# sangminwoo/SVOL

Hardware: AMD Instinct MI355X
Metric: frames/sec (fwd+matcher+bwd), T=32·P=196·d=256 (higher is better)
Workload: dtype bf16

## Files before the change

### svol_amd/csrc/gemm_ws_bf16.hip

```cpp
#include "gemm_call.h"

namespace {

struct WsArgs {
    const h16_t* A; const h16_t* W; void* C;
    const float* bias; const float* colscale; h16_t* pre; const void* res; const h16_t* aux; float* colsum;
    int64_t lda, ldw, ldc, ldp, ldr, ldaux;
    int M, N, act, tiles_per_wg, nchunk;
};

typedef __attribute__((address_space(3))) void* lds_void_ptr;

constexpr int WS_K = 256;
constexpr int TR = 16;
constexpr int A_PLANE = TR * WS_K * 2;

typedef unsigned u32x4_t __attribute__((ext_vector_type(4)));

template <int N> __device__ __forceinline__ void ws_wait_vm() { asm volatile("s_waitcnt vmcnt(%0)" ::"n"(N) : "memory"); }
__device__ __forceinline__ void ws_wait_vm_dyn(int n) {
    switch (n) {
#define C_(x) case x: ws_wait_vm<x>(); break;
        C_(0) C_(1) C_(2) C_(3) C_(4) C_(5) C_(6) C_(7) C_(8) C_(9) C_(10) C_(11) C_(12) C_(13) C_(14) C_(15) C_(16)
        C_(17) C_(18) C_(19) C_(20) C_(21) C_(22) C_(23) C_(24) C_(25) C_(26) C_(27) C_(28) C_(29) C_(30) C_(31) C_(32)
#undef C_
        default: ws_wait_vm<32>(); break;
    }
}

__device__ __forceinline__ int ws_col(int t, int i) { return (t >> 1) * 32 + (i >> 2) * 8 + (t & 1) * 4 + (i & 3); }

template <int MODE> struct WsCfg;
template <> struct WsCfg<0> { static constexpr int SLOT = A_PLANE, STG = 4, ND = 2; };
template <> struct WsCfg<1> { static constexpr int SLOT = A_PLANE + TR * 256 * 4, STG = 3, ND = 6; };
template <> struct WsCfg<2> { static constexpr int SLOT = 2 * A_PLANE, STG = 4, ND = 4; };

template <int MODE>
__device__ __forceinline__ void gemm_ws_body(const WsArgs& p) {
    constexpr int SLOT = WsCfg<MODE>::SLOT, STG = WsCfg<MODE>::STG, ND = WsCfg<MODE>::ND;
    __shared__ __attribute__((aligned(1024))) char smem[STG * SLOT];
    const int tid = threadIdx.x, lane = tid & 63;
    const int wave = __builtin_amdgcn_readfirstlane(tid >> 6);
    const int fr = lane & 15, fq = lane >> 4;
    const int chunk_id = blockIdx.x % p.nchunk, cg = blockIdx.x / p.nchunk;
    const int cg0 = cg * 256;
    const int c0 = cg0 + wave * 64;
    const bool active = c0 < p.N;
    const int tile0 = chunk_id * p.tiles_per_wg;
    const int row_base = tile0 * TR;
    const int rows_here = min(p.tiles_per_wg * TR, p.M - row_base);
    const int ntile = (rows_here + TR - 1) / TR;
    const int ns = !active ? 0 : (MODE == 0 ? (p.pre ? 4 : 2) : (MODE == 1 ? 4 : 2));

    const __amdgpu_buffer_rsrc_t rA = __builtin_amdgcn_make_buffer_rsrc(
        (void*)(p.A + (int64_t)row_base * p.lda), 0, (int)((((int64_t)rows_here - 1) * p.lda + WS_K) * 2), 0x00020000);
    int voffA[2];
#pragma unroll
    for (int j = 0; j < 2; ++j) {
        const int row = (wave * 2 + j) * 2 + (lane >> 5), s = lane & 31;
        voffA[j] = (int)(((int64_t)row * p.lda + ((s ^ row) & 31) * 8) * 2);
    }
    __amdgpu_buffer_rsrc_t rX = rA;
    int voffX[4] = {0, 0, 0, 0};
    if constexpr (MODE == 1) {
        const float* R = reinterpret_cast<const float*>(p.res) + (int64_t)row_base * p.ldr + cg0;
        const int cols = min(256, p.N - cg0);
        rX = __builtin_amdgcn_make_buffer_rsrc((void*)R, 0, (int)((((int64_t)rows_here - 1) * p.ldr + cols) * 4), 0x00020000);
#pragma unroll
        for (int j = 0; j < 4; ++j) {
            const int row = wave * 4 + j, s = lane;
            voffX[j] = (int)(((int64_t)row * p.ldr + (((s & 48) | ((s ^ row) & 15))) * 4) * 4);
        }
    } else if constexpr (MODE == 2) {
        const h16_t* X = p.aux + (int64_t)row_base * p.ldaux + cg0;
        const int cols = min(256, p.N - cg0);
        rX = __builtin_amdgcn_make_buffer_rsrc((void*)X, 0, (int)((((int64_t)rows_here - 1) * p.ldaux + cols) * 2), 0x00020000);
#pragma unroll
        for (int j = 0; j < 2; ++j) {
            const int row = (wave * 2 + j) * 2 + (lane >> 5), s = lane & 31;
            voffX[j] = (int)(((int64_t)row * p.ldaux + ((s ^ row) & 31) * 8) * 2);
        }
    }
    auto issue = [&](int slot, int tile) {
        char* sl = smem + slot * SLOT;
        const int soA = (int)((int64_t)tile * TR * p.lda * 2);
#pragma unroll
        for (int j = 0; j < 2; ++j)
            __builtin_amdgcn_raw_ptr_buffer_load_lds(rA, (lds_void_ptr)(sl + (wave * 2 + j) * 1024), 16, voffA[j], soA, 0, 0);
        if constexpr (MODE == 1) {
            const int so = (int)((int64_t)tile * TR * p.ldr * 4);
#pragma unroll
            for (int j = 0; j < 4; ++j)
                __builtin_amdgcn_raw_ptr_buffer_load_lds(rX, (lds_void_ptr)(sl + A_PLANE + (wave * 4 + j) * 1024), 16, voffX[j], so, 0, 0);
        } else if constexpr (MODE == 2) {
            const int so = (int)((int64_t)tile * TR * p.ldaux * 2);
#pragma unroll
            for (int j = 0; j < 2; ++j)
                __builtin_amdgcn_raw_ptr_buffer_load_lds(rX, (lds_void_ptr)(sl + A_PLANE + (wave * 2 + j) * 1024), 16, voffX[j], so, 0, 0);
        }
    };

    uint4 wf[4][8];
#pragma unroll
    for (int t = 0; t < 4; ++t) {
        const h16_t* wrow = p.W + (int64_t)(c0 + ws_col(t, fr)) * p.ldw + fq * 8;
#pragma unroll
        for (int ks = 0; ks < 8; ++ks) wf[t][ks] = active ? *reinterpret_cast<const uint4*>(wrow + ks * 32) : make_uint4(0, 0, 0, 0);
    }
    float bias8[2][8], scale8[2][8];
#pragma unroll
    for (int hf = 0; hf < 2; ++hf)
#pragma unroll
        for (int e = 0; e < 8; ++e) {
            const int n = c0 + hf * 32 + fq * 8 + e;
            bias8[hf][e] = (active && p.bias) ? p.bias[n] : 0.f;
            scale8[hf][e] = (MODE == 0 && active && p.colscale) ? p.colscale[n] : 1.f;
        }
    float csum[2][8];
#pragma unroll
    for (int hf = 0; hf < 2; ++hf)
#pragma unroll
        for (int e = 0; e < 8; ++e) csum[hf][e] = 0.f;

    const unsigned lds0 = (unsigned)(size_t)(lds_void_ptr)smem;
    const unsigned aoff = (unsigned)(fr * 512 + ((fq ^ fr) & 3) * 16);

#pragma unroll
    for (int s = 0; s < STG - 1; ++s)
        if (s < ntile) issue(s, s);

    for (int j = 0; j < ntile; ++j) {
        ws_wait_vm_dyn(ND * min(STG - 2, ntile - 1 - j) + ns * min(j, STG - 1));
        __builtin_amdgcn_s_barrier();
        if (j + STG - 1 < ntile) issue((j + STG - 1) % STG, j + STG - 1);
        const unsigned sl = lds0 + (unsigned)((j % STG) * SLOT);
        uint4 af[8];
        {
            const unsigned b = sl + aoff;
            const unsigned x = (unsigned)((fr & 12) * 16);
            asm volatile(
                "ds_read_b128 %0, %8\n\t"
                "ds_read_b128 %1, %9\n\t"
                "ds_read_b128 %2, %10\n\t"
                "ds_read_b128 %3, %11\n\t"
                "ds_read_b128 %4, %8 offset:256\n\t"
                "ds_read_b128 %5, %9 offset:256\n\t"
                "ds_read_b128 %6, %10 offset:256\n\t"
                "ds_read_b128 %7, %11 offset:256\n\t"
                "s_waitcnt lgkmcnt(0)"
                : "=&v"(af[0]), "=&v"(af[1]), "=&v"(af[2]), "=&v"(af[3]), "=&v"(af[4]), "=&v"(af[5]), "=&v"(af[6]), "=&v"(af[7])
                : "v"(b + ((0u * 64) ^ x)), "v"(b + ((1u * 64) ^ x)), "v"(b + ((2u * 64) ^ x)), "v"(b + ((3u * 64) ^ x))
                : "memory");
        }
        f32x4 acc[4];
#pragma unroll
        for (int t = 0; t < 4; ++t) acc[t] = f32x4{0.f, 0.f, 0.f, 0.f};
#pragma unroll
        for (int ks = 0; ks < 8; ++ks)
#pragma unroll
            for (int t = 0; t < 4; ++t)
                acc[t] = SVOL_MFMA_16x16x32_H16(__builtin_bit_cast(h16x8, wf[t][ks]),
                                                                 __builtin_bit_cast(h16x8, af[ks]), acc[t], 0, 0, 0);
        const int m = row_base + j * TR + fr;
        float v[2][8];
#pragma unroll
        for (int hf = 0; hf < 2; ++hf)
#pragma unroll
            for (int e = 0; e < 8; ++e) v[hf][e] = acc[2 * hf + (e >> 2)][e & 3];
        if constexpr (MODE == 0) {
#pragma unroll
            for (int hf = 0; hf < 2; ++hf)
#pragma unroll
                for (int e = 0; e < 8; ++e) v[hf][e] = (v[hf][e] + bias8[hf][e]) * scale8[hf][e];
            if (active && m < p.M) {
                if (p.pre) {
#pragma unroll
                    for (int hf = 0; hf < 2; ++hf) {
                        h16x8 o;
#pragma unroll
                        for (int e = 0; e < 8; ++e) o[e] = (h16_t)pre_save_fast(v[hf][e], p.act);
                        *reinterpret_cast<h16x8*>(p.pre + (int64_t)m * p.ldp + c0 + hf * 32 + fq * 8) = o;
// ... 106 lines not shown
template <int MODE, int ACT, bool PRE, bool SCALE, int VPM>
__device__ __forceinline__ void gemm_wsp_body(const WsArgs& p) {
    static_assert(MODE == 0 || MODE == 2, "bf16 outputs only");
    constexpr int SLOT = WsCfg<MODE>::SLOT, STG = 4, ND = WsCfg<MODE>::ND;
    constexpr int NS = MODE == 0 ? (PRE ? 4 : 2) : 2;
    __shared__ __attribute__((aligned(1024))) char smem[STG * SLOT];
    const int tid = threadIdx.x, lane = tid & 63;
    const int wave = __builtin_amdgcn_readfirstlane(tid >> 6);
    const int fr = lane & 15, fq = lane >> 4;
    const int chunk_id = blockIdx.x % p.nchunk, cg = blockIdx.x / p.nchunk;
    const int cg0 = cg * 256;
    const int c0 = cg0 + wave * 64;
    const bool active = c0 < p.N;
    const int tile0 = chunk_id * p.tiles_per_wg;
    const int row_base = tile0 * TR;
    const int rows_here = min(p.tiles_per_wg * TR, p.M - row_base);
    const int ntile = (rows_here + TR - 1) / TR;

    const __amdgpu_buffer_rsrc_t rA = __builtin_amdgcn_make_buffer_rsrc(
        (void*)(p.A + (int64_t)row_base * p.lda), 0, (int)((((int64_t)rows_here - 1) * p.lda + WS_K) * 2), 0x00020000);
    int voffA[2];
#pragma unroll
    for (int j = 0; j < 2; ++j) {
        const int row = (wave * 2 + j) * 2 + (lane >> 5), s = lane & 31;
        voffA[j] = (int)(((int64_t)row * p.lda + ((s ^ row) & 31) * 8) * 2);
    }
    __amdgpu_buffer_rsrc_t rX = rA;
    int voffX[2] = {0, 0};
    if constexpr (MODE == 2) {
        const h16_t* X = p.aux + (int64_t)row_base * p.ldaux + cg0;
        const int cols = min(256, p.N - cg0);
        rX = __builtin_amdgcn_make_buffer_rsrc((void*)X, 0, (int)((((int64_t)rows_here - 1) * p.ldaux + cols) * 2), 0x00020000);
#pragma unroll
        for (int j = 0; j < 2; ++j) {
            const int row = (wave * 2 + j) * 2 + (lane >> 5), s = lane & 31;
            voffX[j] = (int)(((int64_t)row * p.ldaux + ((s ^ row) & 31) * 8) * 2);
        }
    }
    auto issue = [&](int slot, int tile) {
        char* sl = smem + slot * SLOT;
        const int soA = (int)((int64_t)tile * TR * p.lda * 2);
#pragma unroll
        for (int j = 0; j < 2; ++j)
            __builtin_amdgcn_raw_ptr_buffer_load_lds(rA, (lds_void_ptr)(sl + (wave * 2 + j) * 1024), 16, voffA[j], soA, 0, 0);
        if constexpr (MODE == 2) {
            const int so = (int)((int64_t)tile * TR * p.ldaux * 2);
#pragma unroll
            for (int j = 0; j < 2; ++j)
                __builtin_amdgcn_raw_ptr_buffer_load_lds(rX, (lds_void_ptr)(sl + A_PLANE + (wave * 2 + j) * 1024), 16, voffX[j], so, 0, 0);
        }
    };

    uint4 wf[4][8];
#pragma unroll
    for (int t = 0; t < 4; ++t) {
        const h16_t* wrow = p.W + (int64_t)(c0 + ws_col(t, fr)) * p.ldw + fq * 8;
#pragma unroll
        for (int ks = 0; ks < 8; ++ks) wf[t][ks] = active ? *reinterpret_cast<const uint4*>(wrow + ks * 32) : make_uint4(0, 0, 0, 0);
    }
    float bias8[2][8], scale8[2][8];
#pragma unroll
    for (int hf = 0; hf < 2; ++hf)
#pragma unroll
        for (int e = 0; e < 8; ++e) {
            const int n = c0 + hf * 32 + fq * 8 + e;
            bias8[hf][e] = (MODE == 0 && active && p.bias) ? p.bias[n] : 0.f;
            scale8[hf][e] = (MODE == 0 && SCALE && active && p.colscale) ? p.colscale[n] : 1.f;
        }
    float csum[2][8];
#pragma unroll
    for (int hf = 0; hf < 2; ++hf)
#pragma unroll
        for (int e = 0; e < 8; ++e) csum[hf][e] = 0.f;

    const unsigned lds0 = (unsigned)(size_t)(lds_void_ptr)smem;
    const unsigned aoff = (unsigned)(fr * 512 + ((fq ^ fr) & 3) * 16);
    const unsigned ax_x = (unsigned)((fr & 12) * 16);
    const unsigned xq0 = (unsigned)(A_PLANE + fr * 512 + (((wave * 8 + fq) ^ fr) & 31) * 16);
    const unsigned xq1 = (unsigned)(A_PLANE + fr * 512 + (((wave * 8 + 4 + fq) ^ fr) & 31) * 16);
    const __amdgpu_buffer_rsrc_t rC = __builtin_amdgcn_make_buffer_rsrc(
        (void*)(reinterpret_cast<h16_t*>(p.C) + (int64_t)row_base * p.ldc), 0,
        active ? (int)((((int64_t)rows_here - 1) * p.ldc + p.N) * 2) : 0, 0x00020000);
    const __amdgpu_buffer_rsrc_t rP = __builtin_amdgcn_make_buffer_rsrc(
        (void*)(PRE ? p.pre + (int64_t)row_base * p.ldp : nullptr), 0,
        (PRE && active) ? (int)((((int64_t)rows_here - 1) * p.ldp + p.N) * 2) : 0, 0x00020000);
    const int voffC = (int)(((int64_t)fr * p.ldc + c0 + fq * 8) * 2), voffP = (int)(((int64_t)fr * p.ldp + c0 + fq * 8) * 2);
    const int cstep = (int)(TR * p.ldc * 2), pstep = (int)(TR * p.ldp * 2);

    u32x4_t af[8], ax[2] = {u32x4_t{0, 0, 0, 0}, u32x4_t{0, 0, 0, 0}};
    auto read_frags = [&](int slot) {
        const unsigned sl = lds0 + (unsigned)(slot * SLOT);
        const unsigned b = sl + aoff;
        asm volatile(
            "ds_read_b128 %0, %8\n\t"
            "ds_read_b128 %1, %9\n\t"
            "ds_read_b128 %2, %10\n\t"
            "ds_read_b128 %3, %11\n\t"
            "ds_read_b128 %4, %8 offset:256\n\t"
            "ds_read_b128 %5, %9 offset:256\n\t"
            "ds_read_b128 %6, %10 offset:256\n\t"
            "ds_read_b128 %7, %11 offset:256"
            : "=&v"(af[0]), "=&v"(af[1]), "=&v"(af[2]), "=&v"(af[3]), "=&v"(af[4]), "=&v"(af[5]), "=&v"(af[6]), "=&v"(af[7])
            : "v"(b + ((0u * 64) ^ ax_x)), "v"(b + ((1u * 64) ^ ax_x)), "v"(b + ((2u * 64) ^ ax_x)), "v"(b + ((3u * 64) ^ ax_x))
            : "memory");
        if constexpr (MODE == 2) {
            asm volatile(
                "ds_read_b128 %0, %2\n\t"
                "ds_read_b128 %1, %3"
                : "=&v"(ax[0]), "=&v"(ax[1])
                : "v"(sl + xq0), "v"(sl + xq1)
                : "memory");
        }
// ... 15 lines not shown
    };
    auto epilogue = [&](int j, const f32x4 (&acc)[4], const u32x4_t (&axj)[2]) {
        float v[2][8];
#pragma unroll
        for (int hf = 0; hf < 2; ++hf)
#pragma unroll
            for (int e = 0; e < 8; ++e) v[hf][e] = acc[2 * hf + (e >> 2)][e & 3];
        if constexpr (MODE == 0) {
#pragma unroll
            for (int hf = 0; hf < 2; ++hf)
#pragma unroll
                for (int e = 0; e < 8; ++e) {
                    v[hf][e] += bias8[hf][e];
                    if constexpr (SCALE) v[hf][e] *= scale8[hf][e];
                }
            if constexpr (PRE) {
                h16x8 o[2];
#pragma unroll
                for (int hf = 0; hf < 2; ++hf)
#pragma unroll
                    for (int e = 0; e < 8; ++e) o[hf][e] = (h16_t)pre_save_fast(v[hf][e], ACT);
                store_b128_guarded(__builtin_bit_cast(u32x4_t, o[0]), rP, voffP, j * pstep);
                store_b128_guarded(__builtin_bit_cast(u32x4_t, o[1]), rP, voffP + 64, j * pstep);
            }
            h16x8 o[2];
#pragma unroll
            for (int hf = 0; hf < 2; ++hf)
#pragma unroll
                for (int e = 0; e < 8; ++e) {
                    float y = v[hf][e];
                    if constexpr (ACT == SVOL_ACT_GELU || ACT == SVOL_ACT_GELU_D) y = gelu_fast(y);
                    if constexpr (ACT == SVOL_ACT_RELU) y = fmaxf(y, 0.f);
                    o[hf][e] = (h16_t)y;
                }
            store_b128_guarded(__builtin_bit_cast(u32x4_t, o[0]), rC, voffC, j * cstep);
            store_b128_guarded(__builtin_bit_cast(u32x4_t, o[1]), rC, voffC + 64, j * cstep);
        } else {
            h16x8 o[2];
#pragma unroll
            for (int hf = 0; hf < 2; ++hf) {
                const h16x8 a8 = __builtin_bit_cast(h16x8, axj[hf]);
#pragma unroll
                for (int e = 0; e < 8; ++e) {
                    const float d = v[hf][e] * dact_fast((float)a8[e], ACT);
                    csum[hf][e] += d;
                    o[hf][e] = (h16_t)d;
                }
            }
            store_b128_guarded(__builtin_bit_cast(u32x4_t, o[0]), rC, voffC, j * cstep);
            store_b128_guarded(__builtin_bit_cast(u32x4_t, o[1]), rC, voffC + 64, j * cstep);
        }
    };

#pragma unroll
    for (int s = 0; s < STG; ++s)
        if (s < ntile) issue(s, s);
    ws_wait_vm_dyn(ND * min(STG - 1, ntile - 1));
    __builtin_amdgcn_s_barrier();
    read_frags(0);
    wait_frags();
    f32x4 acc[4];
    mfma_slab(acc);
    for (int j = 0; j + 1 < ntile; ++j) {
        const int nd = min(STG - 2, ntile - 2 - j), nst = min(j, STG - 1);
        if (nd == STG - 2 && nst == STG - 1) ws_wait_vm<ND * (STG - 2) + NS * (STG - 1)>();
        else ws_wait_vm_dyn(ND * nd + NS * nst);
        __builtin_amdgcn_s_barrier();
        if (j + STG < ntile) issue(j % STG, j + STG);
        f32x4 accp[4];
        u32x4_t axp[2];
#pragma unroll
        for (int t = 0; t < 4; ++t) accp[t] = acc[t];
        axp[0] = ax[0];
        axp[1] = ax[1];
        read_frags((j + 1) % STG);
        wait_frags();
        mfma_slab(acc);
        epilogue(j, accp, axp);
#pragma unroll
        for (int i = 0; i < 32; ++i) {
            __builtin_amdgcn_sched_group_barrier(0x008, 1, 0);
            __builtin_amdgcn_sched_group_barrier(0x002, VPM, 0);
        }
    }
    {
        u32x4_t axp[2] = {ax[0], ax[1]};
        epilogue(ntile - 1, acc, axp);
    }
    if constexpr (MODE == 2) {
        if (p.colsum) {
#pragma unroll
            for (int hf = 0; hf < 2; ++hf)
#pragma unroll
                for (int e = 0; e < 8; ++e) {
                    float s = csum[hf][e];
                    s += __shfl_xor(s, 1, 64);
                    s += __shfl_xor(s, 2, 64);
                    s += __shfl_xor(s, 4, 64);
                    s += __shfl_xor(s, 8, 64);
                    if (fr == 0 && active) atomicAdd(p.colsum + c0 + hf * 32 + fq * 8 + e, s);
                }
        }
    }
}

#define WSP_KERNEL(name, MODE, ACT, PRE, SCALE, VPM) \
    __global__ __launch_bounds__(256, 2) void name(WsArgs p) { gemm_wsp_body<MODE, ACT, PRE, SCALE, VPM>(p); }
WSP_KERNEL(gemm_wsp_bf16_none, 0, SVOL_ACT_NONE, false, false, 2)
WSP_KERNEL(gemm_wsp_bf16_none_scale, 0, SVOL_ACT_NONE, false, true, 2)
WSP_KERNEL(gemm_wsp_bf16_gelu, 0, SVOL_ACT_GELU, false, false, 7)
WSP_KERNEL(gemm_wsp_bf16_gelu_pre, 0, SVOL_ACT_GELU, true, false, 8)
WSP_KERNEL(gemm_wsp_bf16_gelu_dpre, 0, SVOL_ACT_GELU_D, true, false, 9)
WSP_KERNEL(gemm_wsp_bf16_relu, 0, SVOL_ACT_RELU, false, false, 2)
WSP_KERNEL(gemm_wsp_bf16_dgelu, 2, SVOL_ACT_GELU, false, false, 9)
WSP_KERNEL(gemm_wsp_bf16_dmul, 2, SVOL_ACT_GELU_D, false, false, 3)
WSP_KERNEL(gemm_wsp_bf16_drelu, 2, SVOL_ACT_RELU, false, false, 3)
#undef WSP_KERNEL

}

static int ws_plan(const GemmCall& c, WsArgs& p, dim3& grid, void (*&kern)(WsArgs)) {
    const int64_t M = c.M, N = c.N;
    const int act = c.act;
    if (c.kwrap != c.K || c.K != WS_K || N % 64 || M < 4096) return SVOL_E_UNSUPPORTED;
    int mode;
    if (c.epi == 1) {
        if (!c.aux || c.out_f32) return SVOL_E_UNSUPPORTED;
        mode = 2;
    } else if (c.out_f32) {
        if (!c.res || act != SVOL_ACT_NONE || c.pre || c.colscale) return SVOL_E_UNSUPPORTED;
        mode = 1;
    } else {
        if (c.res || (act != SVOL_ACT_NONE && act != SVOL_ACT_GELU && act != SVOL_ACT_RELU && act != SVOL_ACT_GELU_D)) return SVOL_E_UNSUPPORTED;
        if (act == SVOL_ACT_GELU_D && !c.pre) return SVOL_E_INVALID;
        mode = 0;
    }
    if (c.lda % 8 || c.ldb % 8 || !aligned16(c.A) || !aligned16(c.B) || !aligned16(c.C)) return SVOL_E_UNSUPPORTED;
    if (mode == 1 ? (c.ldc % 4 || c.ldr % 4 || !aligned16(c.res)) : (c.ldc % 8 != 0)) return SVOL_E_UNSUPPORTED;
    if (c.pre && (c.ldp % 8 || !aligned16(c.pre))) return SVOL_E_UNSUPPORTED;
    if (mode == 2 && (c.ldaux % 8 || !aligned16(c.aux))) return SVOL_E_UNSUPPORTED;
    const int64_t ntile = (M + TR - 1) / TR;
    const int64_t ncg = (N + 255) / 256;
    int64_t tpw = (ntile * ncg + (ncg <= 2 ? 255 : 511)) / (ncg <= 2 ? 256 : 512);
    if (tpw < 4) tpw = 4;
    if (tpw > 64) tpw = 64;
    const int64_t ldmax = c.lda > c.ldr * 2 ? c.lda : c.ldr * 2;
    int64_t ldbig = ldmax > c.ldaux ? ldmax : c.ldaux;
    if (c.ldc > ldbig) ldbig = c.ldc;
    if (c.pre && c.ldp > ldbig) ldbig = c.ldp;
    if (tpw * TR * ldbig * 2 >= (1ll << 31)) return SVOL_E_UNSUPPORTED;
    int64_t nchunk = (ntile + tpw - 1) / tpw;
    if (ncg > 1 && nchunk > 8 && nchunk % 8) {
        const int64_t n8 = (nchunk + 7) / 8 * 8;
        const int64_t t8 = (ntile + n8 - 1) / n8;
        if (t8 >= 1 && (ntile + t8 - 1) / t8 == n8) { tpw = t8; nchunk = n8; }
    }
    if (nchunk * ncg > (1ll << 30)) return SVOL_E_UNSUPPORTED;
    p = WsArgs{(const h16_t*)c.A, (const h16_t*)c.B, c.C, c.bias, c.colscale, (h16_t*)c.pre, c.res, (const h16_t*)c.aux, c.colsum,
               c.lda, c.ldb, c.ldc, c.ldp, c.ldr, c.ldaux, (int)M, (int)N, act, (int)tpw, (int)nchunk};
    grid = dim3((unsigned)(ncg * nchunk));
    kern = mode == 0 ? gemm_ws_bf16_m0 : (mode == 1 ? gemm_ws_bf16_m1 : gemm_ws_bf16_m2);
    if (mode == 0) {
        if (act == SVOL_ACT_NONE && !c.pre) kern = c.colscale ? gemm_wsp_bf16_none_scale : gemm_wsp_bf16_none;
        else if (act == SVOL_ACT_GELU && !c.colscale) kern = c.pre ? gemm_wsp_bf16_gelu_pre : gemm_wsp_bf16_gelu;
        else if (act == SVOL_ACT_GELU_D && !c.colscale) kern = gemm_wsp_bf16_gelu_dpre;
        else if (act == SVOL_ACT_RELU && !c.pre && !c.colscale) kern = gemm_wsp_bf16_relu;
    } else if (mode == 2) {
        kern = act == SVOL_ACT_RELU ? gemm_wsp_bf16_drelu : (act == SVOL_ACT_GELU_D ? gemm_wsp_bf16_dmul : gemm_wsp_bf16_dgelu);
    }
    return SVOL_OK;
}

int svol_gemm_ws_bf16(const GemmCall& c) {
    WsArgs p; dim3 grid; void (*kern)(WsArgs);
    if (const int rc = ws_plan(c, p, grid, kern)) return rc;
    hipLaunchKernelGGL(kern, grid, dim3(256), 0, c.stream, p);
    return hipGetLastError() == hipSuccess ? SVOL_OK : SVOL_E_LAUNCH;
}
```

### svol_amd/csrc/norm.hip

```cpp
#include "common.h"

namespace {

constexpr int LN_MAX_PASSES = 4;

template <typename T, typename TX, int NP>
__global__ __launch_bounds__(256) void ln_fwd_kernel(const TX* __restrict__ x, const float* __restrict__ gamma,
                                                     const float* __restrict__ beta, float* __restrict__ y32,
                                                     T* __restrict__ y, T* __restrict__ ypos, const T* __restrict__ pos,
                                                     int64_t pos_rows, float* __restrict__ mean, float* __restrict__ rstd,
                                                     int64_t M, int D, float p, float inv_keep, uint64_t seed0,
                                                     const int64_t* __restrict__ soff) {
    const uint64_t seed = seed0 + (soff ? ((uint64_t)soff[0] << 8) : 0ull);
    const int lane = threadIdx.x & 63;
    const int64_t row = (int64_t)blockIdx.x * 4 + (threadIdx.x >> 6);
    if (row >= M) return;
    const TX* xr = x + row * D;
    float v[NP][4];
    float s = 0.f;
    const T* pr = pos ? pos + (row % pos_rows) * D : nullptr;
    Vec4<TX> t[NP];
    Vec4<T> pv[NP];
    Vec4<float> gv[NP], bv[NP];
#pragma unroll
    for (int j = 0; j < NP; ++j) {
        const int c = (lane + 64 * j) * 4;
        if (c < D) {
            t[j].load(xr + c);
            if (pr) pv[j].load(pr + c);
            gv[j].load(gamma + c);
            bv[j].load(beta + c);
        }
    }
#pragma unroll
    for (int j = 0; j < NP; ++j) {
        const int c = (lane + 64 * j) * 4;
#pragma unroll
        for (int e = 0; e < 4; ++e) {
            v[j][e] = c < D ? t[j].get(e) : 0.f;
            s += v[j][e];
        }
    }
    const float mu = wave_sum(s) / (float)D;
    float q = 0.f;
#pragma unroll
    for (int j = 0; j < NP; ++j) {
        const int c = (lane + 64 * j) * 4;
        if (c < D) {
#pragma unroll
            for (int e = 0; e < 4; ++e) { const float d = v[j][e] - mu; q += d * d; }
        }
    }
    const float rs = rsqrtf(wave_sum(q) / (float)D + 1e-5f);
    if (lane == 0) { mean[row] = mu; rstd[row] = rs; }
#pragma unroll
    for (int j = 0; j < NP; ++j) {
        const int c = (lane + 64 * j) * 4;
        if (c < D) {
            Vec4<T> o, op;
            Vec4<float> o32;
#pragma unroll
            for (int e = 0; e < 4; ++e) {
                float r = (v[j][e] - mu) * rs * gv[j].get(e) + bv[j].get(e);
                if (p > 0.f) r *= dropout_scale(seed, (uint64_t)row, (uint32_t)(c + e), p, inv_keep);
                o.set(e, r);
                o32.set(e, r);
                if (pr) op.set(e, r + pv[j].get(e));
            }
            if (y32) o32.store(y32 + row * D + c);
            if (y) o.store(y + row * D + c);
            if (ypos) op.store(ypos + row * D + c);
        }
    }
}

template <typename T, typename TX, int NP>
__global__ __launch_bounds__(256) void ln_bwd_kernel(const float* __restrict__ dy32, const T* __restrict__ dy,
                                                     const T* __restrict__ dy2, const TX* __restrict__ x,
                                                     const float* __restrict__ gamma, const float* __restrict__ mean,
                                                     const float* __restrict__ rstd, float* __restrict__ dx32,
                                                     T* __restrict__ dx, float* __restrict__ dgamma,
                                                     float* __restrict__ dbeta, float* __restrict__ dxsum, int64_t M, int D,
                                                     float p, float inv_keep, uint64_t seed0, const int64_t* __restrict__ soff, int rows_per_wave,
                                                     float* __restrict__ det_part) {
    const uint64_t seed = seed0 + (soff ? ((uint64_t)soff[0] << 8) : 0ull);
    const int lane = threadIdx.x & 63;
    const int64_t wave_id = (int64_t)blockIdx.x * 4 + (threadIdx.x >> 6);
    const int64_t r0 = wave_id * rows_per_wave;
    float dg[NP][4], db[NP][4], dxs[NP][4], gm[NP][4];
#pragma unroll
    for (int j = 0; j < NP; ++j) {
        const int c = (lane + 64 * j) * 4;
#pragma unroll
        for (int e = 0; e < 4; ++e) { dg[j][e] = 0.f; db[j][e] = 0.f; dxs[j][e] = 0.f; gm[j][e] = c < D ? gamma[c + e] : 0.f; }
    }
    struct Row { Vec4<float> a32[NP]; Vec4<T> a[NP], b[NP]; Vec4<TX> xv[NP]; float mu, rs; };
    auto fetch = [&](int64_t row, Row& r) {
#pragma unroll
        for (int j = 0; j < NP; ++j) {
            const int c = (lane + 64 * j) * 4;
            if (c < D) {
                if (dy32) r.a32[j].load(dy32 + row * D + c);
                if (dy) r.a[j].load(dy + row * D + c);
                if (dy2) r.b[j].load(dy2 + row * D + c);
                r.xv[j].load(x + row * D + c);
            }
        }
        r.mu = mean[row];
        r.rs = rstd[row];
    };
    const int64_t rend = (r0 + rows_per_wave < M) ? r0 + rows_per_wave : M;
    Row cur, nxt;
    if (r0 < rend) fetch(r0, cur);
    for (int64_t row = r0; row < rend; ++row) {
        if (row + 1 < rend) fetch(row + 1, nxt);
        const float mu = cur.mu, rs = cur.rs;
        float g[NP][4], xh[NP][4];
        float s1 = 0.f, s2 = 0.f;
#pragma unroll
        for (int j = 0; j < NP; ++j) {
            const int c = (lane + 64 * j) * 4;
            if (c < D) {
#pragma unroll
                for (int e = 0; e < 4; ++e) {
                    float d = (dy32 ? cur.a32[j].get(e) : 0.f) + (dy ? cur.a[j].get(e) : 0.f) + (dy2 ? cur.b[j].get(e) : 0.f);
                    if (p > 0.f) d *= dropout_scale(seed, (uint64_t)row, (uint32_t)(c + e), p, inv_keep);
                    const float h = (cur.xv[j].get(e) - mu) * rs;
                    xh[j][e] = h;
                    dg[j][e] += d * h;
                    db[j][e] += d;
                    const float gg = d * gm[j][e];
                    g[j][e] = gg;
                    s1 += gg;
                    s2 += gg * h;
                }
            }
        }
        s1 = wave_sum(s1) / (float)D;
        s2 = wave_sum(s2) / (float)D;
#pragma unroll
        for (int j = 0; j < NP; ++j) {
            const int c = (lane + 64 * j) * 4;
            if (c < D) {
                Vec4<T> o;
                Vec4<float> o32;
#pragma unroll
                for (int e = 0; e < 4; ++e) {
                    const float r = rs * (g[j][e] - s1 - xh[j][e] * s2);
                    dxs[j][e] += r;
                    o.set(e, r);
                    o32.set(e, r);
                }
                if (dx32) o32.store(dx32 + row * D + c);
                if (dx) o.store(dx + row * D + c);
            }
        }
        cur = nxt;
    }
    __shared__ float red[3][NP * 256];
    const int wave = threadIdx.x >> 6;
    for (int w = 0; w < 4; ++w) {
        if (wave == w) {
#pragma unroll
            for (int j = 0; j < NP; ++j) {
                const int c = (lane + 64 * j) * 4;
                if (c < D) {
#pragma unroll
                    for (int e = 0; e < 4; ++e) {
                        if (w == 0) { red[0][c + e] = dg[j][e]; red[1][c + e] = db[j][e]; red[2][c + e] = dxs[j][e]; }
                        else { red[0][c + e] += dg[j][e]; red[1][c + e] += db[j][e]; red[2][c + e] += dxs[j][e]; }
                    }
                }
            }
        }
        __syncthreads();
    }
    if (det_part) {
        float* row = det_part + (int64_t)blockIdx.x * 3 * D;
        for (int c = threadIdx.x; c < D; c += 256) { row[c] = red[0][c]; row[D + c] = red[1][c]; row[2 * D + c] = red[2][c]; }
        return;
    }
    for (int c = threadIdx.x; c < D; c += 256) {
        atomicAdd(dgamma + c, red[0][c]);
        atomicAdd(dbeta + c, red[1][c]);
        if (dxsum) atomicAdd(dxsum + c, red[2][c]);
    }
}

template <typename T>
__global__ __launch_bounds__(256) void posenc_kernel(const float* __restrict__ mask, T* __restrict__ pos, int L, int D) {
    __shared__ float red[2][4];
    __shared__ float xe[64];
    const int b = blockIdx.y, tid = threadIdx.x, lane = tid & 63, wave = tid >> 6;
    const float* mr = mask + (int64_t)b * L;
    const int l0 = blockIdx.x * 64;
    float before = 0.f, all = 0.f;
    for (int l = tid; l < L; l += 256) {
        const float v = (mr[l] != 0.f) ? 1.f : 0.f;
        all += v;
        if (l < l0) before += v;
    }
    before = wave_sum(before);
    all = wave_sum(all);
    if (lane == 0) { red[0][wave] = before; red[1][wave] = all; }
    __syncthreads();
    if (tid == 0) {
        float run = red[0][0] + red[0][1] + red[0][2] + red[0][3];
// ... 52 lines not shown
        int64_t r = i / row_len;
        int64_t k = i - r * row_len;
        uint32_t rm = drop_row(s0, (uint64_t)r);
#pragma unroll
        for (int e = 0; e < 4; ++e) {
            if (i + e >= n) break;
            out[i + e] = res[i + e] + t[i + e] * drop_scale_rk(rm, (uint32_t)k, p, inv_keep);
            if (++k == row_len) { k = 0; ++r; rm = drop_row(s0, (uint64_t)r); }
        }
    }
}
}

extern "C" {

int svol_layernorm_fwd(const void* x, int x_f32, const float* gamma, const float* beta, float* y32, void* y,
                       void* ypos, const void* pos, int64_t pos_rows, float* mean, float* rstd, int64_t M, int64_t D,
                       float dropout_p, uint64_t seed, const int64_t* seed_offset_dev, int dtype, void* stream) {
    if (!x || !gamma || !beta || (!y && !y32) || !mean || !rstd || M < 0 || D <= 0) return SVOL_E_INVALID;
    if (!aligned16(gamma) || !aligned16(beta)) return SVOL_E_INVALID;
    if ((ypos != nullptr) != (pos != nullptr)) return SVOL_E_INVALID;
    if (pos && pos_rows <= 0) return SVOL_E_INVALID;
    if (D % 4 || D > LN_MAX_PASSES * 256) return SVOL_E_UNSUPPORTED;
    if (dropout_p < 0.f || dropout_p >= 1.f) return SVOL_E_INVALID;
    if (!svol_is16(dtype) && dtype != SVOL_F32) return SVOL_E_INVALID;
    if (M == 0) return SVOL_OK;
    const float inv_keep = 1.f / (1.f - dropout_p);
    const unsigned grid = (unsigned)((M + 3) / 4);
    hipStream_t s = reinterpret_cast<hipStream_t>(stream);
#define SVOL_LNF(TT, TXX, NPP)                                                                                              \
    hipLaunchKernelGGL((ln_fwd_kernel<TT, TXX, NPP>), dim3(grid), dim3(256), 0, s, (const TXX*)x, gamma, beta, y32, (TT*)y,      \
                       (TT*)ypos, (const TT*)pos, pos_rows, mean, rstd, M, (int)D, dropout_p, inv_keep, seed, seed_offset_dev)
#define SVOL_LNF_NP(TT, TXX)                     \
    do {                                         \
        if (D <= 256) SVOL_LNF(TT, TXX, 1);      \
        else if (D <= 512) SVOL_LNF(TT, TXX, 2); \
        else SVOL_LNF(TT, TXX, 4);               \
    } while (0)
    if (dtype == SVOL_BF16 && x_f32) SVOL_LNF_NP(bf16_t, float);
    else if (dtype == SVOL_BF16) SVOL_LNF_NP(bf16_t, bf16_t);
    else if (dtype == SVOL_F16 && x_f32) SVOL_LNF_NP(f16_t, float);
    else if (dtype == SVOL_F16) SVOL_LNF_NP(f16_t, f16_t);
    else SVOL_LNF_NP(float, float);
#undef SVOL_LNF_NP
#undef SVOL_LNF
    SVOL_CHECK_LAUNCH();
    return SVOL_OK;
}

int svol_layernorm_bwd(const float* dy32, const void* dy, const void* dy2, const void* x, int x_f32, const float* gamma,
                       const float* mean, const float* rstd, float* dx32, void* dx, float* dgamma, float* dbeta,
                       float* dx_colsum, int64_t M, int64_t D, float dropout_p, uint64_t seed, const int64_t* seed_offset_dev,
                       int dtype, void* stream) {
    if ((!dy32 && !dy && !dy2) || !x || !gamma || !mean || !rstd || (!dx && !dx32) || !dgamma || !dbeta || M < 0 || D <= 0)
        return SVOL_E_INVALID;
    if (D % 4 || D > LN_MAX_PASSES * 256) return SVOL_E_UNSUPPORTED;
    if (dropout_p < 0.f || dropout_p >= 1.f) return SVOL_E_INVALID;
    if (!svol_is16(dtype) && dtype != SVOL_F32) return SVOL_E_INVALID;
    if (M == 0) return SVOL_OK;
    const float inv_keep = 1.f / (1.f - dropout_p);
    int64_t rpw = (M + 2047) / 2048;
    if (rpw < 1) rpw = 1;
    const int64_t waves = (M + rpw - 1) / rpw;
    const unsigned grid = (unsigned)((waves + 3) / 4);
    hipStream_t s = reinterpret_cast<hipStream_t>(stream);
    const bool det_mode = svol_deterministic();
    DetScratch det(det_mode ? (size_t)grid * 3 * (size_t)D : 0, s);
    if (det_mode && !det.p) return SVOL_E_LAUNCH;
#define SVOL_LNB(TT, TXX, NPP)                                                                                                      \
    hipLaunchKernelGGL((ln_bwd_kernel<TT, TXX, NPP>), dim3(grid), dim3(256), 0, s, dy32, (const TT*)dy, (const TT*)dy2, (const TXX*)x, \
                       gamma, mean, rstd, dx32, (TT*)dx, dgamma, dbeta, dx_colsum, M, (int)D, dropout_p, inv_keep, seed,              \
                       seed_offset_dev, (int)rpw, det.p)
#define SVOL_LNB_NP(TT, TXX)                  \
    do {                                      \
        if (D <= 256) SVOL_LNB(TT, TXX, 1);   \
        else if (D <= 512) SVOL_LNB(TT, TXX, 2); \
        else SVOL_LNB(TT, TXX, 4);            \
    } while (0)
    if (dtype == SVOL_BF16 && x_f32) SVOL_LNB_NP(bf16_t, float);
    else if (dtype == SVOL_BF16) SVOL_LNB_NP(bf16_t, bf16_t);
    else if (dtype == SVOL_F16 && x_f32) SVOL_LNB_NP(f16_t, float);
    else if (dtype == SVOL_F16) SVOL_LNB_NP(f16_t, f16_t);
    else SVOL_LNB_NP(float, float);
#undef SVOL_LNB_NP
#undef SVOL_LNB
    if (det_mode) {
        det_fold(det.p, (int)grid, 3 * D, dgamma, D, s);
        det_fold(det.p + D, (int)grid, 3 * D, dbeta, D, s);
        det_fold(det.p + 2 * D, (int)grid, 3 * D, dx_colsum, D, s);
    }
    SVOL_CHECK_LAUNCH();
    return SVOL_OK;
}

int svol_dropout_sd(const void* x, void* y, int64_t n, int64_t row_len, float p, uint64_t seed, const int64_t* seed_step_dev, int dtype,
                    void* stream) {
    if (!x || !y || n < 0 || row_len <= 0 || row_len > 0xffffffffll || !(p >= 0.f && p < 1.f)) return SVOL_E_INVALID;
    if (n == 0) return SVOL_OK;
    const float inv = 1.f / (1.f - p);
    int64_t g = (n + 1023) / 1024;
    if (g > 8192) g = 8192;
    hipStream_t s = reinterpret_cast<hipStream_t>(stream);
    if (dtype == SVOL_F32) hipLaunchKernelGGL(dropout_kernel<float>, dim3((unsigned)g), dim3(256), 0, s, (const float*)x, (float*)y, n, row_len, p, inv, seed, seed_step_dev);
    else if (dtype == SVOL_BF16) hipLaunchKernelGGL(dropout_kernel<bf16_t>, dim3((unsigned)g), dim3(256), 0, s, (const bf16_t*)x, (bf16_t*)y, n, row_len, p, inv, seed, seed_step_dev);
    else if (dtype == SVOL_F16) hipLaunchKernelGGL(dropout_kernel<f16_t>, dim3((unsigned)g), dim3(256), 0, s, (const f16_t*)x, (f16_t*)y, n, row_len, p, inv, seed, seed_step_dev);
    else return SVOL_E_INVALID;
    SVOL_CHECK_LAUNCH();
    return SVOL_OK;
}

int svol_dropout(const void* x, void* y, int64_t n, int64_t row_len, float p, uint64_t seed, int dtype, void* stream) {
    return svol_dropout_sd(x, y, n, row_len, p, seed, nullptr, dtype, stream);
}

int svol_dropout_add_sd(const float* t32, const float* res32, float* out32, int64_t n, int64_t row_len, float p, uint64_t seed,
                        const int64_t* seed_step_dev, void* stream) {
    if (!t32 || !res32 || !out32 || n < 0 || row_len <= 0 || row_len > 0xffffffffll || !(p >= 0.f && p < 1.f)) return SVOL_E_INVALID;
    if (n == 0) return SVOL_OK;
    int64_t g = (n + 1023) / 1024;
    if (g > 8192) g = 8192;
    hipLaunchKernelGGL(dropout_add_kernel, dim3((unsigned)g), dim3(256), 0, reinterpret_cast<hipStream_t>(stream), t32, res32, out32, n,
                       row_len, p, 1.f / (1.f - p), seed, seed_step_dev);
    SVOL_CHECK_LAUNCH();
    return SVOL_OK;
}
int svol_dropout_add(const float* t32, const float* res32, float* out32, int64_t n, int64_t row_len, float p, uint64_t seed, void* stream) {
    return svol_dropout_add_sd(t32, res32, out32, n, row_len, p, seed, nullptr, stream);
}

int svol_posenc_sine(const float* mask, void* pos, int64_t B, int64_t L, int64_t D, int dtype, void* stream) {
    if (!mask || !pos || B <= 0 || L <= 0 || D <= 0) return SVOL_E_INVALID;
    if (L > (1 << 24) || D > 4096) return SVOL_E_UNSUPPORTED;
    hipStream_t s = reinterpret_cast<hipStream_t>(stream);
    if (B > 65535) return SVOL_E_UNSUPPORTED;
    dim3 grid((unsigned)((L + 63) / 64), (unsigned)B);
    if (dtype == SVOL_BF16)
        hipLaunchKernelGGL(posenc_kernel<bf16_t>, grid, dim3(256), 0, s, mask, (bf16_t*)pos, (int)L, (int)D);
    else if (dtype == SVOL_F16)
// ... 10 lines not shown
```

### svol_amd/layers.py

```python
from __future__ import annotations

import math
import os

import torch

from . import _lib
from .ops import (ACT_GELU, ACT_NONE, ACT_RELU, _DT, _ptr, _stream, act_bwd, attn_bwd, attn_fwd, attn_weights_mean, cast, colsum,
                  dropout, dropout_add, gemm_nt, gemm_nt_dact, gemm_nt_split, layernorm_bwd, layernorm_fwd)
from .params import SPLIT_V, GradGroup, claim, sink_view, unless_sunk, weights


def _pos_grad(dypos, pos_shape, D):
    rows = 1
    for n in pos_shape[:-1]:
        rows *= n
    g = colsum(dypos.reshape(-1, rows * D).contiguous())
    return cast(g.view(pos_shape), dypos.dtype)


class LayerNormFn(torch.autograd.Function):

    @staticmethod
    def forward(ctx, x, gamma, beta, p, seed, seed_dev):
        shp = x.shape
        x2 = x.reshape(-1, shp[-1])
        _, y, _, mean, rstd = layernorm_fwd(x2, gamma, beta, x.dtype, None, p, seed, seed_dev=seed_dev)
        ctx.save_for_backward(x2, gamma, mean, rstd, seed_dev)
        ctx.p, ctx.seed, ctx.shp = p, seed, shp
        ctx.sinks = (claim(gamma, ctx.needs_input_grad[1]), claim(beta, ctx.needs_input_grad[2]))
        return y.view(shp)

    @staticmethod
    def backward(ctx, dy):
        x2, gamma, mean, rstd, seed_dev = ctx.saved_tensors
        sg, sb = ctx.sinks
        _, dx, dg, db = layernorm_bwd(None, dy, None, x2, gamma, mean, rstd, x2.dtype, ctx.p, ctx.seed, seed_dev=seed_dev,
                                      dg_out=sink_view(sg), db_out=sink_view(sb))
        return dx.view(ctx.shp), unless_sunk(sg, dg), unless_sunk(sb, db), None, None, None


def layer_norm(x, gamma, beta, p=0.0, seed=0, seed_dev=None):
    return LayerNormFn.apply(x, gamma, beta, p, seed, seed_dev)


class LinearFn(torch.autograd.Function):

    @staticmethod
    def forward(ctx, x, W, b, act, out_f32):
        if act == ACT_GELU:
            raise _lib.SvolHipError('LinearFn: GELU is only available fused in MLPLNFn')
        shp = x.shape
        x2 = x.reshape(-1, shp[-1])
        Wc, WcT = weights.get(W, x.dtype)
        y = gemm_nt(x2, Wc, b, act, out_f32=out_f32)
        ctx.save_for_backward(x2, y if act != ACT_NONE else None)
        ctx.WcT, ctx.act, ctx.shp, ctx.has_b = WcT, act, shp, b is not None
        ctx.need_dx = ctx.needs_input_grad[0]
        epc = 4 if x.dtype == torch.float32 else 8
        ok = W.shape[0] % epc == 0
        ctx.sinks = (claim(W, ok and ctx.needs_input_grad[1]), claim(b, ok and ctx.needs_input_grad[2]))
        return y.view(*shp[:-1], W.shape[0])

    @staticmethod
    def backward(ctx, dy):
        x2, y = ctx.saved_tensors
        N = dy.shape[-1]
        d = dy.reshape(-1, N)
        if not d.is_contiguous():
            d = d.contiguous()
        if d.dtype != x2.dtype:
            d = cast(d, x2.dtype)
        if ctx.act != ACT_NONE:
            d = act_bwd(d, y, ctx.act)
        epc = 4 if d.dtype == torch.float32 else 8
        WcT = ctx.WcT
        Np = (N + epc - 1) // epc * epc
        if N % epc:
            dp = torch.zeros((d.shape[0], Np), dtype=d.dtype, device=d.device)
            dp[:, :N] = d
            wp = torch.zeros((WcT.shape[0], Np), dtype=WcT.dtype, device=WcT.device)
            wp[:, :N] = WcT
            d, WcT = dp, wp
        K_ = x2.shape[1]
        sW, sb = ctx.sinks
        grads = GradGroup(((sW, (Np, K_)), (sb, (Np,), ctx.has_b)), d.device)
        grads.tn(d, x2, 0, 1 if ctx.has_b else None)
        dW, db = grads.finish()
        if N != Np:
            dW, db = dW[:N], db[:N] if ctx.has_b else None
        dx = gemm_nt(d, WcT).view(ctx.shp) if ctx.need_dx else None
        return dx, dW, db, None, None
# ... 504 lines not shown
```

### svol_amd/ops.py

```python
from __future__ import annotations

import ctypes
import math
import os
from typing import Optional

import torch

from . import _lib, wgrad

ACT_NONE, ACT_RELU, ACT_GELU, ACT_SIGMOID, ACT_RELU_RES, ACT_GELU_D = 0, 1, 2, 3, 4, 5
_DT = {torch.float32: 0, torch.bfloat16: 1, torch.float16: 2}


def _dt(t: torch.Tensor) -> int:
    try:
        return _DT[t.dtype]
    except KeyError:
        raise _lib.SvolHipError(f'unsupported dtype {t.dtype}')


_RAW_STREAM = getattr(torch._C, '_cuda_getCurrentRawStream', None)
_CUR_DEVICE = getattr(torch._C, '_cuda_getDevice', None)

# ... 162 lines not shown
                                      aux.stride(0), act, _ptr(cs), M, N, K, _dt(A), _stream())
    _lib.check(rc, 'svol_gemm_nt_dact')
    return out, cs


def gemm_nt_dgelu(A, B, pre, want_colsum=True, colsum_out=None):
    return gemm_nt_dact(A, B, pre, ACT_GELU, want_colsum, colsum_out)


def colsum(X, out=None):
    assert X.dim() == 2 and X.stride(1) == 1
    M, N = X.shape
    if out is None:
        out = torch.zeros((N,), dtype=torch.float32, device=X.device)
    _lib.check(_lib.lib().svol_colsum(_ptr(X), X.stride(0), _ptr(out), M, N, _dt(X), _stream()), 'svol_colsum')
    return out


def act_bwd(dy, aux, act):
    dy = dy.contiguous()
    aux = aux.contiguous()
    out = torch.empty_like(dy)
    _lib.check(_lib.lib().svol_act_bwd(_ptr(dy), _ptr(aux), _ptr(out), act, dy.numel(), _dt(dy), _stream()),
               'svol_act_bwd')
    return out


def layernorm_fwd(x, gamma, beta, dtype, pos=None, p=0.0, seed=0, want32=False, want_t=True, seed_dev=None):
    x = x.contiguous()
    M, D = x.shape
    x_f32 = 1 if (x.dtype == torch.float32 and dtype != torch.float32) else 0
    assert x.dtype in (dtype, torch.float32)
    y32 = torch.empty((M, D), dtype=torch.float32, device=x.device) if want32 else None
    y = torch.empty((M, D), dtype=dtype, device=x.device) if want_t else None
    ypos = torch.empty((M, D), dtype=dtype, device=x.device) if pos is not None else None
    mean = torch.empty((M,), dtype=torch.float32, device=x.device)
    rstd = torch.empty((M,), dtype=torch.float32, device=x.device)
    if pos is not None:
        pos = pos.contiguous()
        assert pos.dtype == dtype and pos.shape[-1] == D
    rc = _lib.lib().svol_layernorm_fwd(_ptr(x), x_f32, _ptr(gamma), _ptr(beta), _ptr(y32), _ptr(y), _ptr(ypos),
                                       _ptr(pos), pos.numel() // D if pos is not None else 0, _ptr(mean), _ptr(rstd),
                                       M, D, float(p), int(seed), _ptr(seed_dev), _DT[dtype], _stream())
    _lib.check(rc, 'svol_layernorm_fwd')
    return y32, y, ypos, mean, rstd


def layernorm_bwd(dy32, dy, dy2, x, gamma, mean, rstd, dtype, p=0.0, seed=0, want32=False, want_t=True,
                  want_colsum=False, seed_dev=None, dg_out=None, db_out=None, cs_out=None):
    M, D = x.shape
    x_f32 = 1 if (x.dtype == torch.float32 and dtype != torch.float32) else 0
    cont = lambda t: None if t is None else t.reshape(M, D).contiguous()
    dy32, dy, dy2 = cont(dy32), cont(dy), cont(dy2)
    assert dy32 is None or dy32.dtype == torch.float32
    assert (dy is None or dy.dtype == dtype) and (dy2 is None or dy2.dtype == dtype)
    dx32 = torch.empty((M, D), dtype=torch.float32, device=x.device) if want32 else None
    dx = torch.empty((M, D), dtype=dtype, device=x.device) if want_t else None
    dg, db, cs = dg_out, db_out, (cs_out if want_colsum else None)
    if dg is None or db is None or (want_colsum and cs is None):
        red = torch.zeros((3, D), dtype=torch.float32, device=x.device)
        dg = red[0] if dg is None else dg
        db = red[1] if db is None else db
        cs = (red[2] if cs is None else cs) if want_colsum else None
    rc = _lib.lib().svol_layernorm_bwd(_ptr(dy32), _ptr(dy), _ptr(dy2), _ptr(x), x_f32, _ptr(gamma), _ptr(mean),
                                       _ptr(rstd), _ptr(dx32), _ptr(dx), _ptr(dg), _ptr(db), _ptr(cs), M, D, float(p),
                                       int(seed), _ptr(seed_dev), _DT[dtype], _stream())
    _lib.check(rc, 'svol_layernorm_bwd')
    if want_colsum:
        return dx32, dx, dg, db, cs
    return dx32, dx, dg, db


def posenc_sine(mask_f32: torch.Tensor, D: int, dtype: torch.dtype) -> torch.Tensor:
    mask_f32 = mask_f32.contiguous()
    B, L = mask_f32.shape
    pos = torch.empty((B, L, D), dtype=dtype, device=mask_f32.device)
    _lib.check(_lib.lib().svol_posenc_sine(_ptr(mask_f32), _ptr(pos), B, L, D, _DT[dtype], _stream()),
               'svol_posenc_sine')
    return pos


def attn_ws_bytes(dtype, B, H, Lq, Lk, dh):
    return max(int(_lib.lib().svol_attn_ws_bytes(B, H, Lq, Lk, dh)), 0) if dtype != torch.float32 else 0


def _attn_ws(q, B, H, Lq, Lk, dh):
    n = attn_ws_bytes(q.dtype, B, H, Lq, Lk, dh)
    return torch.empty((n // 4,), dtype=torch.float32, device=q.device) if n else None


def dropout(x, p, seed, out=None, seed_dev=None):
    assert x.is_contiguous()
    out = torch.empty_like(x) if out is None else out
    args = (_ptr(x), _ptr(out), x.numel(), max(1, x.shape[-1] if x.dim() else 1), float(p), int(seed))
    if seed_dev is None:
        _lib.check(_lib.lib().svol_dropout(*args, _dt(x), _stream()), 'svol_dropout')
    else:
        _lib.check(_lib.lib().svol_dropout_sd(*args, _ptr(seed_dev), _dt(x), _stream()), 'svol_dropout_sd')
    return out


def dropout_add(t32, res32, p, seed, seed_dev=None):
    assert t32.is_contiguous() and res32.is_contiguous() and t32.dtype == torch.float32 and res32.dtype == torch.float32
    args = (_ptr(t32), _ptr(res32), _ptr(t32), t32.numel(), max(1, t32.shape[-1]), float(p), int(seed))
    if seed_dev is None:
        _lib.check(_lib.lib().svol_dropout_add(*args, _stream()), 'svol_dropout_add')
# ... 289 lines not shown
```

Baseline: 15220.

## Stage GEMM weight loads through LDS with async buffer loads; skip unneeded LN dx

Weight fragments for the weight-stationary GEMM kernels are now loaded asynchronously into LDS with buffer_load_lds in double-buffered halves, then read into registers with swizzled ds_reads. The first A-tile prefetches are issued during the last weight half so they overlap. This replaces the per-thread strided global loads of the weights. Separately, the LayerNorm backward gains a compile-time path that skips computing and storing dx when autograd does not need the input gradient, saving the reduction and the write. The cost is a more complex prologue and a new guard on the weight buffer size.

```diff
diff --git a/svol_amd/csrc/gemm_ws_bf16.hip b/svol_amd/csrc/gemm_ws_bf16.hip
--- a/svol_amd/csrc/gemm_ws_bf16.hip
+++ b/svol_amd/csrc/gemm_ws_bf16.hip
@@ -34,6 +34,58 @@
 template <> struct WsCfg<0> { static constexpr int SLOT = A_PLANE, STG = 4, ND = 2; };
 template <> struct WsCfg<1> { static constexpr int SLOT = A_PLANE + TR * 256 * 4, STG = 3, ND = 6; };
 template <> struct WsCfg<2> { static constexpr int SLOT = 2 * A_PLANE, STG = 4, ND = 4; };
+
+template <int MODE, typename F>
+__device__ __forceinline__ void ws_load_w(uint4 (&wf)[4][8], const WsArgs& p, char* smem, int wave, int lane, int c0, int n_early,
+                                          F&& issue_early) {
+    constexpr int SLOT = WsCfg<MODE>::SLOT, STG = WsCfg<MODE>::STG;
+    const int fr = lane & 15, fq = lane >> 4;
+    auto piece = [&](int r, int q) -> int {
+        if constexpr (STG == 4) return (2 * r + (q >> 1)) * SLOT + (wave * 2 + (q & 1)) * 1024;
+        else return r * SLOT + (q < 2 ? (wave * 2 + q) * 1024 : A_PLANE + (wave * 4 + q - 2) * 1024);
+    };
+    const __amdgpu_buffer_rsrc_t rW =
+        __builtin_amdgcn_make_buffer_rsrc((void*)p.W, 0, (int)((((int64_t)p.N - 1) * p.ldw + WS_K) * 2), 0x00020000);
+    int voffW[4];
+#pragma unroll
+    for (int i = 0; i < 4; ++i) {
+        const int row = 4 * i + (lane >> 4), s = lane & 15;
+        voffW[i] = (int)(((int64_t)(c0 + ws_col(0, row)) * p.ldw + ((s ^ row) & 15) * 8) * 2);
+    }
+    auto issue_w = [&](int h) {
+        const int t = h >> 1, kh = h & 1;
+        const int so = (int)(((int64_t)ws_col(t, 0) * p.ldw + kh * 128) * 2);
+#pragma unroll
+        for (int i = 0; i < 4; ++i)
+            __builtin_amdgcn_raw_ptr_buffer_load_lds(rW, (lds_void_ptr)(smem + piece(h & 1, i)), 16, voffW[i], so, 0, 0);
+    };
+    const unsigned lds0 = (unsigned)(size_t)(lds_void_ptr)smem;
+    unsigned rd[2];
+#pragma unroll
+    for (int r = 0; r < 2; ++r) rd[r] = lds0 + (unsigned)(piece(r, fr >> 2) + (fr & 3) * 256 + ((fq ^ fr) & 3) * 16);
+    const unsigned kx = (unsigned)(fr >> 2);
+    issue_w(0);
+    issue_w(1);
+#pragma unroll
+    for (int h = 0; h < 8; ++h) {
+        if (h < 7) ws_wait_vm<4>();
+        else ws_wait_vm_dyn(n_early);
+        const unsigned b = rd[h & 1];
+        uint4(&w)[8] = wf[h >> 1];
+        const int k0 = (h & 1) * 4;
+        asm volatile(
+            "ds_read_b128 %0, %4\n\t"
+            "ds_read_b128 %1, %5\n\t"
+            "ds_read_b128 %2, %6\n\t"
+            "ds_read_b128 %3, %7\n\t"
+            "s_waitcnt lgkmcnt(0)"
+            : "=&v"(w[k0]), "=&v"(w[k0 + 1]), "=&v"(w[k0 + 2]), "=&v"(w[k0 + 3])
+            : "v"(b + ((0u ^ kx) * 64)), "v"(b + ((1u ^ kx) * 64)), "v"(b + ((2u ^ kx) * 64)), "v"(b + ((3u ^ kx) * 64))
+            : "memory");
+        if (h + 2 < 8) issue_w(h + 2);
+        if (h == 6) issue_early();
+    }
+}
 
 template <int MODE>
 __device__ __forceinline__ void gemm_ws_body(const WsArgs& p) {
@@ -101,12 +153,6 @@
     };
 
     uint4 wf[4][8];
-#pragma unroll
-    for (int t = 0; t < 4; ++t) {
-        const h16_t* wrow = p.W + (int64_t)(c0 + ws_col(t, fr)) * p.ldw + fq * 8;
-#pragma unroll
-        for (int ks = 0; ks < 8; ++ks) wf[t][ks] = active ? *reinterpret_cast<const uint4*>(wrow + ks * 32) : make_uint4(0, 0, 0, 0);
-    }
     float bias8[2][8], scale8[2][8];
 #pragma unroll
     for (int hf = 0; hf < 2; ++hf)
@@ -125,8 +171,14 @@
     const unsigned lds0 = (unsigned)(size_t)(lds_void_ptr)smem;
     const unsigned aoff = (unsigned)(fr * 512 + ((fq ^ fr) & 3) * 16);
 
-#pragma unroll
-    for (int s = 0; s < STG - 1; ++s)
+    constexpr int EARLY = STG == 4 ? 2 : 1;
+    ws_load_w<MODE>(wf, p, smem, wave, lane, c0, ND * min(EARLY, ntile), [&]() {
+#pragma unroll
+        for (int s = 0; s < EARLY; ++s)
+            if (s < ntile) issue(s, s);
+    });
+#pragma unroll
+    for (int s = EARLY; s < STG - 1; ++s)
         if (s < ntile) issue(s, s);
 
     for (int j = 0; j < ntile; ++j) {
@@ -339,12 +391,6 @@
     };
 
     uint4 wf[4][8];
-#pragma unroll
-    for (int t = 0; t < 4; ++t) {
-        const h16_t* wrow = p.W + (int64_t)(c0 + ws_col(t, fr)) * p.ldw + fq * 8;
-#pragma unroll
-        for (int ks = 0; ks < 8; ++ks) wf[t][ks] = active ? *reinterpret_cast<const uint4*>(wrow + ks * 32) : make_uint4(0, 0, 0, 0);
-    }
     float bias8[2][8], scale8[2][8];
 #pragma unroll
     for (int hf = 0; hf < 2; ++hf)
@@ -466,8 +512,13 @@
         }
     };
 
-#pragma unroll
-    for (int s = 0; s < STG; ++s)
+    ws_load_w<MODE>(wf, p, smem, wave, lane, c0, ND * min(2, ntile), [&]() {
+#pragma unroll
+        for (int s = 0; s < 2; ++s)
+            if (s < ntile) issue(s, s);
+    });
+#pragma unroll
+    for (int s = 2; s < STG; ++s)
         if (s < ntile) issue(s, s);
     ws_wait_vm_dyn(ND * min(STG - 1, ntile - 1));
     __builtin_amdgcn_s_barrier();
@@ -563,6 +614,7 @@
     if (c.ldc > ldbig) ldbig = c.ldc;
     if (c.pre && c.ldp > ldbig) ldbig = c.ldp;
     if (tpw * TR * ldbig * 2 >= (1ll << 31)) return SVOL_E_UNSUPPORTED;
+    if ((ncg * 256 * c.ldb + WS_K) * 2 >= (1ll << 31)) return SVOL_E_UNSUPPORTED;
     int64_t nchunk = (ntile + tpw - 1) / tpw;
     if (ncg > 1 && nchunk > 8 && nchunk % 8) {
         const int64_t n8 = (nchunk + 7) / 8 * 8;
diff --git a/svol_amd/csrc/norm.hip b/svol_amd/csrc/norm.hip
--- a/svol_amd/csrc/norm.hip
+++ b/svol_amd/csrc/norm.hip
@@ -74,7 +74,7 @@
     }
 }
 
-template <typename T, typename TX, int NP>
+template <typename T, typename TX, int NP, bool WANT_DX>
 __global__ __launch_bounds__(256) void ln_bwd_kernel(const float* __restrict__ dy32, const T* __restrict__ dy,
                                                      const T* __restrict__ dy2, const TX* __restrict__ x,
                                                      const float* __restrict__ gamma, const float* __restrict__ mean,
@@ -136,23 +136,25 @@
                 }
             }
         }
-        s1 = wave_sum(s1) / (float)D;
-        s2 = wave_sum(s2) / (float)D;
-#pragma unroll
-        for (int j = 0; j < NP; ++j) {
-            const int c = (lane + 64 * j) * 4;
-            if (c < D) {
-                Vec4<T> o;
-                Vec4<float> o32;
-#pragma unroll
-                for (int e = 0; e < 4; ++e) {
-                    const float r = rs * (g[j][e] - s1 - xh[j][e] * s2);
-                    dxs[j][e] += r;
-                    o.set(e, r);
-                    o32.set(e, r);
+        if constexpr (WANT_DX) {
+            s1 = wave_sum(s1) / (float)D;
+            s2 = wave_sum(s2) / (float)D;
+#pragma unroll
+            for (int j = 0; j < NP; ++j) {
+                const int c = (lane + 64 * j) * 4;
+                if (c < D) {
+                    Vec4<T> o;
+                    Vec4<float> o32;
+#pragma unroll
+                    for (int e = 0; e < 4; ++e) {
+                        const float r = rs * (g[j][e] - s1 - xh[j][e] * s2);
+                        dxs[j][e] += r;
+                        o.set(e, r);
+                        o32.set(e, r);
+                    }
+                    if (dx32) o32.store(dx32 + row * D + c);
+                    if (dx) o.store(dx + row * D + c);
                 }
-                if (dx32) o32.store(dx32 + row * D + c);
-                if (dx) o.store(dx + row * D + c);
             }
         }
         cur = nxt;
@@ -311,8 +313,10 @@
                        const float* mean, const float* rstd, float* dx32, void* dx, float* dgamma, float* dbeta,
                        float* dx_colsum, int64_t M, int64_t D, float dropout_p, uint64_t seed, const int64_t* seed_offset_dev,
                        int dtype, void* stream) {
-    if ((!dy32 && !dy && !dy2) || !x || !gamma || !mean || !rstd || (!dx && !dx32) || !dgamma || !dbeta || M < 0 || D <= 0)
+    if ((!dy32 && !dy && !dy2) || !x || !gamma || !mean || !rstd || !dgamma || !dbeta || M < 0 || D <= 0)
         return SVOL_E_INVALID;
+    const bool want_dx = dx || dx32;
+    if (!want_dx && dx_colsum) return SVOL_E_INVALID;
     if (D % 4 || D > LN_MAX_PASSES * 256) return SVOL_E_UNSUPPORTED;
     if (dropout_p < 0.f || dropout_p >= 1.f) return SVOL_E_INVALID;
     if (!svol_is16(dtype) && dtype != SVOL_F32) return SVOL_E_INVALID;
@@ -326,10 +330,15 @@
     const bool det_mode = svol_deterministic();
     DetScratch det(det_mode ? (size_t)grid * 3 * (size_t)D : 0, s);
     if (det_mode && !det.p) return SVOL_E_LAUNCH;
-#define SVOL_LNB(TT, TXX, NPP)                                                                                                      \
-    hipLaunchKernelGGL((ln_bwd_kernel<TT, TXX, NPP>), dim3(grid), dim3(256), 0, s, dy32, (const TT*)dy, (const TT*)dy2, (const TXX*)x, \
-                       gamma, mean, rstd, dx32, (TT*)dx, dgamma, dbeta, dx_colsum, M, (int)D, dropout_p, inv_keep, seed,              \
+#define SVOL_LNB_DX(TT, TXX, NPP, DXX)                                                                                                    \
+    hipLaunchKernelGGL((ln_bwd_kernel<TT, TXX, NPP, DXX>), dim3(grid), dim3(256), 0, s, dy32, (const TT*)dy, (const TT*)dy2, (const TXX*)x, \
+                       gamma, mean, rstd, dx32, (TT*)dx, dgamma, dbeta, dx_colsum, M, (int)D, dropout_p, inv_keep, seed,                   \
                        seed_offset_dev, (int)rpw, det.p)
+#define SVOL_LNB(TT, TXX, NPP)                      \
+    do {                                            \
+        if (want_dx) SVOL_LNB_DX(TT, TXX, NPP, true); \
+        else SVOL_LNB_DX(TT, TXX, NPP, false);      \
+    } while (0)
 #define SVOL_LNB_NP(TT, TXX)                  \
     do {                                      \
         if (D <= 256) SVOL_LNB(TT, TXX, 1);   \
@@ -343,6 +352,7 @@
     else SVOL_LNB_NP(float, float);
 #undef SVOL_LNB_NP
 #undef SVOL_LNB
+#undef SVOL_LNB_DX
     if (det_mode) {
         det_fold(det.p, (int)grid, 3 * D, dgamma, D, s);
         det_fold(det.p + D, (int)grid, 3 * D, dbeta, D, s);
diff --git a/svol_amd/layers.py b/svol_amd/layers.py
--- a/svol_amd/layers.py
+++ b/svol_amd/layers.py
@@ -35,9 +35,10 @@
     def backward(ctx, dy):
         x2, gamma, mean, rstd, seed_dev = ctx.saved_tensors
         sg, sb = ctx.sinks
-        _, dx, dg, db = layernorm_bwd(None, dy, None, x2, gamma, mean, rstd, x2.dtype, ctx.p, ctx.seed, seed_dev=seed_dev,
-                                      dg_out=sink_view(sg), db_out=sink_view(sb))
-        return dx.view(ctx.shp), unless_sunk(sg, dg), unless_sunk(sb, db), None, None, None
+        need_dx = ctx.needs_input_grad[0]
+        _, dx, dg, db = layernorm_bwd(None, dy, None, x2, gamma, mean, rstd, x2.dtype, ctx.p, ctx.seed, want_t=need_dx,
+                                      seed_dev=seed_dev, dg_out=sink_view(sg), db_out=sink_view(sb))
+        return dx.view(ctx.shp) if need_dx else None, unless_sunk(sg, dg), unless_sunk(sb, db), None, None, None
 
 
 def layer_norm(x, gamma, beta, p=0.0, seed=0, seed_dev=None):
diff --git a/svol_amd/ops.py b/svol_amd/ops.py
--- a/svol_amd/ops.py
+++ b/svol_amd/ops.py
@@ -238,6 +238,7 @@
     x_f32 = 1 if (x.dtype == torch.float32 and dtype != torch.float32) else 0
     cont = lambda t: None if t is None else t.reshape(M, D).contiguous()
     dy32, dy, dy2 = cont(dy32), cont(dy), cont(dy2)
+    assert want32 or want_t or not want_colsum
     assert dy32 is None or dy32.dtype == torch.float32
     assert (dy is None or dy.dtype == dtype) and (dy2 is None or dy2.dtype == dtype)
     dx32 = torch.empty((M, D), dtype=torch.float32, device=x.device) if want32 else None
```

Result: no change. 15240 (median of 3 runs) (+0.1%).
